# 1275468127/Medical-SAM2

Measured on AMD Instinct MI355X. Metric: slices/sec @1024^2 (Hiera-S), higher is better.
Workload: dtype bf16; 1 GPU; configs[1]: sam2_hiera_s 2D (train_2d SAM2 sub-sequence, forward), b=4 x 1024x1024 per GPU, 16-entry memory bank with 4 sampled memories per slice, one click per slice; forward_image -> memory_attention -> prompt encoder -> mask decoder -> memory encoder; hip_graph=True, weights=random name-keyed init

## Files before the change

include/msam2_hip.h:

```cpp
#ifndef MSAM2_HIP_H
#define MSAM2_HIP_H

#include <stddef.h>
#include <stdint.h>

#ifdef __cplusplus
extern "C" {
#endif

const char* msam2_last_error(void);

int msam2_version(void);

int msam2_operand_is_fp16(void);

int msam2_graph_begin(void* stream);

int msam2_graph_end(void* stream, void** graph_exec_out);

int msam2_graph_launch(void* graph_exec, void* stream);

int msam2_graph_destroy(void* graph_exec);

int msam2_event_create(void** ev);
// ... 71 lines not shown
int msam2_bilinear_upsample(const float* x, float* y, int64_t planes, int64_t h, int64_t w, int64_t H, int64_t W, void* stream);

int msam2_sine_pos_2d(float* out, int64_t h, int64_t w, int64_t C, float temperature, void* stream);

int msam2_fourier_pe_grid(float* out, const float* gauss, int64_t h, int64_t w, int64_t C, void* stream);

int msam2_hiera_pos_embed(float* out, const float* pos_embed, const float* pos_embed_window, int64_t C, int64_t bh, int64_t bw, int64_t h, int64_t w, int64_t window, void* stream);

int msam2_aa_downsample(const float* x, float* y, int64_t planes, int64_t H, int64_t W, int64_t factor, float in_scale, float in_bias, void* stream);

int msam2_gate_rows(float* x, const float* score, float value, int64_t B, int64_t row_len, void* stream);

int msam2_any_positive(const float* x, float* out, int64_t B, int64_t row_len, void* stream);

int msam2_image_prep(const uint8_t* img_hwc, float* out_chw, int64_t H, int64_t W, int64_t S, const float* mean3, const float* std3, void* stream);

int msam2_non_overlap(const float* masks, float* out, int64_t n_obj, int64_t pixels, void* stream);

int msam2_seg_counts(const float* pred, const float* gt, const float* thresholds, int64_t n_thresholds, int64_t planes, int64_t pixels, int* counts, void* stream);

int msam2_im2col_patch7x7s4(const float* img, void* out, int64_t B, int64_t S, void* stream);

int msam2_patch_embed7x7s4(const float* img, const void* w_perm, const float* bias, const float* pos, float* out, int64_t B, int64_t S, int64_t E, void* stream);

int msam2_im2col3x3s2(const void* x, void* out, int64_t B, int64_t H, int64_t W, int64_t C, int64_t ld, void* stream);

int msam2_conv3x3s2_ln_gelu(const void* x, int in_is_16bit, const float* weight, const float* bias, const float* ln_w, const float* ln_b, void* y, int64_t B, int64_t H, int64_t W, int64_t Cin, int64_t Cout, int mask_mode, float mask_scale, float mask_bias, void* stream);

int msam2_dwconv7x7_ln(const float* x, const float* weight_tap_major, const float* bias, const float* ln_w, const float* ln_b, void* y, int64_t B, int64_t H, int64_t W, int64_t C, void* stream);

int msam2_convt2x2_shuffle(const void* gemm_out, const float* bias, const void* skip, const float* ln_w, const float* ln_b, void* y, int64_t B, int64_t h, int64_t w, int64_t C, void* stream);

int msam2_convt2x2_shuffle_f32skip(const void* gemm_out, const float* bias, const float* skip, const float* ln_w, const float* ln_b, void* y, int64_t B, int64_t h, int64_t w, int64_t C, void* stream);

int msam2_convt2x2_shuffle_shared(const void* gemm_out, const float* bias, const void* skip, int skip_is_16bit, const float* ln_w, const float* ln_b, void* y, int64_t B, int64_t h, int64_t w, int64_t C, int64_t skip_batch_stride, void* stream);

int msam2_hyper_masks(const float* hyper, const void* upscaled, float* masks, int64_t n, int64_t K, int64_t P, int64_t C, void* stream);

int msam2_prompt_points(const float* xy, const int* labels, const float* gauss, const float* point_emb, const float* not_a_point, float* out, int64_t n_points, int64_t C, float image_size, void* stream);

int msam2_prompt_points_padded(const float* xy, const int* labels, const float* gauss, const float* point_emb, const float* not_a_point, float* out, int64_t n_sets, int64_t P, int64_t n_pad, int64_t C, float image_size, void* stream);

int msam2_select_mask(const float* masks, const float* ious, const float* obj_scores, float* low_res, int* sel, float* iou_sel, int64_t n, int64_t P, int multimask, int dynamic_stability, float delta, float thresh, void* stream);

int msam2_gather_rows(const float* x, const int* sel, float* y, int64_t n, int64_t T, int64_t C, int64_t offset, void* stream);

int msam2_obj_ptr_mix(float* ptr, const float* obj_scores, const float* no_obj_ptr, int64_t n, int64_t C, void* stream);

int msam2_space_to_depth(const void* x, int in_is_16bit, void* out, int64_t B, int64_t H, int64_t W, int64_t C, int64_t k, int64_t ld, void* stream);

int msam2_token_mlp3(const float* hs, int64_t hs_batch_stride, int64_t hs_token_stride, const int* token_index, const void* w1, const float* b1, const void* w2, const float* b2, const void* w3, const float* b3, const int* out_dim, const int* sigmoid_flag, float* out, int64_t G, int64_t B, int64_t C, void* stream);

int msam2_token_mlp3_packed(const float* hs, int64_t hs_batch_stride, int64_t hs_token_stride, const int* token_index, const void* w1, const float* b1, const void* w2, const float* b2, const void* w3, const float* b3, const int* out_dim, const int* sigmoid_flag, float* out, const int* out_offset, const int* out_stride, int64_t G, int64_t B, int64_t C, void* stream);

size_t msam2_cc_workspace_bytes(int64_t N, int64_t H, int64_t W);

int msam2_cc_label(const uint8_t* img, int32_t* labels, int32_t* counts, int64_t N, int64_t H, int64_t W, void* workspace, size_t workspace_bytes, void* stream);

size_t msam2_fill_holes_workspace_bytes(int64_t N, int64_t H, int64_t W);

int msam2_fill_components(float* mask, int64_t N, int64_t H, int64_t W, int max_area, float threshold, int above, float fill_value, void* workspace, size_t workspace_bytes, void* stream);

int msam2_fill_holes(float* mask, int64_t N, int64_t H, int64_t W, int max_area, void* workspace, size_t workspace_bytes, void* stream);

int msam2_transpose16(const void* in, int64_t ldi, void* out, int64_t ldo, int64_t rows, int64_t cols, void* stream);

int msam2_gemm_tt(const void* A, int64_t lda, const void* B, int64_t ldb, float* C, int64_t ldc, float* a_colsum, int64_t M, int64_t N, int64_t K, void* stream);

int msam2_gemm_tt_acc(const void* A, int64_t lda, const void* B, int64_t ldb, float* C, int64_t ldc, float* a_colsum, int64_t M, int64_t N, int64_t K, void* stream);

int msam2_colsum(const void* x, int x_is_16bit, int64_t ldx, float* out, int64_t rows, int64_t cols, void* stream);

int msam2_act_bwd(const void* pre, int pre_is_16bit, const void* dy, int dy_is_16bit, void* out, int64_t n, int act, void* stream);

int msam2_layernorm_bwd(const float* x, int64_t ldx, const void* dy, int dy_is_16bit, int64_t ldd, const float* gamma, float* dx, int64_t ldo, float* dgamma, float* dbeta, int64_t rows, int64_t C, float eps, const float* add, int64_t ld_add, void* stream);

int msam2_softmax_rows(const float* s, int64_t ld_s, void* p, int64_t ld_p, int64_t rows, int64_t cols, float scale, void* stream);

int msam2_softmax_bwd_rows(const void* p, int64_t ld_p, const float* dp, int64_t ld_dp, void* ds, int64_t ld_ds, int64_t rows, int64_t cols, float scale, void* stream);

int msam2_convt2x2_gather(const void* gemm_out, const float* bias, const void* skip, float* z, int64_t B, int64_t h, int64_t w, int64_t C, void* stream);

int msam2_convt2x2_scatter_grad(const void* dz, int dz_is_16bit, void* dg, int64_t B, int64_t h, int64_t w, int64_t C, void* stream);

int msam2_dwconv7x7(const float* x, const float* w_tap_major, const float* bias, float* y, int64_t B, int64_t H, int64_t W, int64_t C, int flip, void* stream);

int msam2_dwconv7x7_wgrad(const float* x, const float* dy, float* dw_tap_major, int64_t B, int64_t H, int64_t W, int64_t C, void* stream);

int msam2_col2im3x3s2(const float* dcols, int64_t ld, float* dx, int64_t B, int64_t H, int64_t W, int64_t C, void* stream);

int msam2_bilinear_upsample_bwd(const float* dy, float* dx, int64_t planes, int64_t h, int64_t w, int64_t H, int64_t W, void* stream);

int msam2_bce_logits(const float* logits, const float* target, float* dlogits, float* loss, int64_t n, float pos_weight, void* stream);

int msam2_adam_step(float* param, const float* grad, float* exp_avg, float* exp_avg_sq, int64_t n, float lr, float beta1, float beta2, float eps, int64_t step, void* stream);

int msam2_adam_step_multi(void* const* params, const void* const* grads, void* const* exp_avg, void* const* exp_avg_sq, const int64_t* numel, int64_t count, float lr, float beta1, float beta2, float eps, int64_t step, float grad_scale, float weight_decay, void* step_counter, void* skipped_counter, void* stream);

int msam2_attention_small_bwd(const void* q, int64_t q_bs, int64_t q_ts, const void* k, int64_t k_bs, int64_t k_ts, const void* v, int64_t v_bs, int64_t v_ts, const float* d_o, float* dq, float* dk, float* dv, int64_t B, int64_t H, int64_t Lq, int64_t Lk, int64_t D, float scale, void* stream);

int msam2_maxpool2x2_bwd(const void* x, int x_is_16bit, int64_t ldx, const float* dy, int64_t lddy, float* dx, int64_t lddx, int64_t B, int64_t H, int64_t W, int64_t C, void* stream);

int msam2_window_move(void* img, int64_t ld_img, void* win, const void* fill, int64_t B, int64_t H, int64_t W, int64_t heads, int64_t D, int64_t ws, int elem_bytes, int to_windows, void* stream);

int msam2_window_unpartition_cvt(void* img16, int64_t ld_img, const float* win, int64_t B, int64_t H, int64_t W, int64_t heads, int64_t D, int64_t ws, void* stream);

// ... 95 lines not shown
```

medical-sam2_amd/_lib.py:

```python
from __future__ import annotations

import ctypes
import os
import subprocess

_HERE = os.path.dirname(os.path.abspath(__file__))
LIB_PATH = os.environ.get("MSAM2_LIB_PATH") or os.path.join(_HERE, "libmsam2_hip.so")

c_p = ctypes.c_void_p
c_i = ctypes.c_int
c_l = ctypes.c_int64
c_f = ctypes.c_float
c_z = ctypes.c_size_t
c_d = ctypes.c_double

SIGNATURES = {
    "msam2_version": (c_i, []),
    "msam2_last_error": (ctypes.c_char_p, []),
    "msam2_operand_is_fp16": (c_i, []),
    "msam2_gemm": (c_i, [c_p, c_l, c_p, c_l, c_p, c_p, c_p, c_l, c_i, c_l, c_p, c_l, c_i, c_l, c_l, c_l, c_i, c_p]),
    "msam2_gemm_pool2x2": (c_i, [c_p, c_l, c_p, c_l, c_p, c_p, c_l, c_l, c_l, c_l, c_l, c_l, c_p]),
    "msam2_gemm_qkv_pool2x2": (c_i, [c_p, c_l, c_p, c_l, c_p, c_p, c_l, c_p, c_l, c_l, c_l, c_l, c_l, c_l, c_l, c_p]),
    "msam2_gemm_tokens": (c_i, [c_p, c_l, c_p, c_l, c_p, c_l, c_p, c_p, c_l, c_p, c_l, c_i, c_l, c_l, c_l, c_i, c_p]),
    "msam2_gemm_rope": (c_i, [c_p, c_l, c_p, c_l, c_p, c_p, c_l, c_l, c_l, c_l, c_p, c_p, c_l, c_l, c_l, c_l, c_l, c_p]),
    "msam2_gemm_residual_layernorm_supported": (c_i, [c_l, c_l]),
    "msam2_gemm_residual_layernorm": (c_i, [c_p, c_l, c_p, c_l, c_p, c_p, c_l, c_p, c_l, c_p, c_p, c_f, c_p, c_l, c_l, c_l, c_l, c_p]),
    "msam2_ln_mlp_residual_supported": (c_i, [c_l]),
    "msam2_mlp_fused_permute_w2": (c_i, [c_p, c_p, c_l, c_l, c_p]),
    "msam2_ln_mlp_residual_fwd": (c_i, [c_p, c_l, c_l, c_p, c_p, c_f, c_p, c_p, c_p, c_p, c_p, c_p]),
    "msam2_ln_mlp_residual_fwd_dual": (c_i, [c_p, c_l, c_l, c_p, c_p, c_f, c_p, c_p, c_p, c_p, c_p, c_p, c_p]),
    "msam2_proj_ln_mlp_residual_supported": (c_i, [c_l]),
    "msam2_mlp_fused_permute_w1": (c_i, [c_p, c_p, c_l, c_l, c_p]),
    "msam2_proj_ln_mlp_residual_fwd": (c_i, [c_p, c_p, c_p, c_p, c_l, c_l, c_p, c_p, c_f, c_p, c_p, c_p, c_p, c_p, c_p, c_p, c_p, c_f, c_p, c_p]),
    "msam2_layernorm": (c_i, [c_p, c_i, c_l, c_p, c_p, c_p, c_i, c_l, c_l, c_l, c_f, c_i, c_p]),
    "msam2_layernorm_dual": (c_i, [c_p, c_l, c_p, c_p, c_p, c_l, c_p, c_l, c_l, c_l, c_f, c_p]),
    "msam2_attention_workspace_bytes": (c_z, [c_l, c_l, c_l, c_l, c_i]),
    "msam2_attention_fwd": (c_i, [c_p, c_p, c_p, c_p, c_p, c_p, c_p, c_p, c_l, c_l, c_l, c_l, c_l, c_f, c_i, c_p, c_z, c_p]),
    "msam2_attention_fwd_lse": (c_i, [c_p, c_p, c_p, c_p, c_p, c_p, c_p, c_p, c_l, c_l, c_l, c_l, c_l, c_f, c_i, c_p, c_z, c_p, c_p]),
    "msam2_attention_fwd_lse_dropout": (c_i, [c_p, c_p, c_p, c_p, c_p, c_p, c_p, c_p, c_l, c_l, c_l, c_l, c_l, c_f, c_i, c_p, c_z, c_p, c_f,
                                              ctypes.c_uint64, ctypes.c_uint64, c_p, c_p]),
    "msam2_attention_kv64_fwd": (c_i, [c_p, c_p, c_p, c_p, c_p, c_p, c_p, c_p, c_l, c_l, c_l, c_l, c_f, c_i, c_p, c_z, c_p]),
    "msam2_attention_kv64_partial": (c_i, [c_p, c_p, c_p, c_p, c_p, c_p, c_l, c_l, c_l, c_l, c_f, c_i, c_i, c_i, c_p, c_z, c_p]),
    "msam2_attention_kv64_dyn_fwd": (c_i, [c_p, c_p, c_p, c_p, c_p, c_p, c_p, c_p, c_l, c_l, c_l, c_l, c_p, c_f, c_i, c_p, c_z, c_p]),
    "msam2_attention_kv64_dyn_partial": (c_i, [c_p, c_p, c_p, c_p, c_p, c_p, c_l, c_l, c_l, c_l, c_p, c_f, c_i, c_i, c_i, c_p, c_z, c_p]),
    "msam2_attention_effective_splits": (c_i, [c_l, c_i]),
    "msam2_attention_merge": (c_i, [c_p, c_p, c_l, c_l, c_l, c_l, c_l, c_i, c_p, c_z, c_p]),
    "msam2_window_attention_fwd": (c_i, [c_p, c_l, c_l, c_l, c_l, c_l, c_p, c_p, c_l, c_l, c_l, c_l, c_l, c_p, c_p, c_p, c_l, c_l,
                                         c_l, c_l, c_l, c_f, c_p]),
    "msam2_window_qkv_attention_supported": (c_i, [c_l, c_l, c_l, c_l, c_i, c_l, c_l]),
    "msam2_window_qkv_attention_fwd": (c_i, [c_p, c_p, c_p, c_p, c_l, c_l, c_l, c_l, c_l, c_l, c_i, c_f, c_p]),
    "msam2_attention_small_fwd": (c_i, [c_p, c_l, c_l, c_p, c_l, c_l, c_p, c_l, c_l, c_p, c_l, c_l, c_l, c_l, c_l, c_l, c_l, c_f,
                                        c_p]),
    "msam2_add_cast": (c_i, [c_p, c_i, c_l, c_l, c_p, c_i, c_l, c_l, c_f, c_p, c_i, c_l, c_l, c_l, c_p]),
    "msam2_maxpool2x2": (c_i, [c_p, c_i, c_l, c_p, c_i, c_l, c_l, c_l, c_l, c_l, c_p]),
    "msam2_upsample2x_add": (c_i, [c_p, c_p, c_l, c_l, c_l, c_l, c_p]),
    "msam2_rope_table": (c_i, [c_p, c_p, c_l, c_l, c_f, c_p]),
    "msam2_rope_inplace": (c_i, [c_p, c_l, c_l, c_l, c_l, c_l, c_l, c_l, c_p, c_p, c_p]),
    "msam2_bilinear_upsample": (c_i, [c_p, c_p, c_l, c_l, c_l, c_l, c_l, c_p]),
    "msam2_sine_pos_2d": (c_i, [c_p, c_l, c_l, c_l, c_f, c_p]),
    "msam2_fourier_pe_grid": (c_i, [c_p, c_p, c_l, c_l, c_l, c_p]),
    "msam2_hiera_pos_embed": (c_i, [c_p, c_p, c_p, c_l, c_l, c_l, c_l, c_l, c_l, c_p]),
    "msam2_im2col_patch7x7s4": (c_i, [c_p, c_p, c_l, c_l, c_p]),
    "msam2_patch_embed7x7s4": (c_i, [c_p, c_p, c_p, c_p, c_p, c_l, c_l, c_l, c_p]),
    "msam2_im2col3x3s2": (c_i, [c_p, c_p, c_l, c_l, c_l, c_l, c_l, c_p]),
    "msam2_conv3x3s2_ln_gelu": (c_i, [c_p, c_i, c_p, c_p, c_p, c_p, c_p, c_l, c_l, c_l, c_l, c_l, c_i, c_f, c_f, c_p]),
    "msam2_dwconv7x7_ln": (c_i, [c_p, c_p, c_p, c_p, c_p, c_p, c_l, c_l, c_l, c_l, c_p]),
    "msam2_convt2x2_shuffle": (c_i, [c_p, c_p, c_p, c_p, c_p, c_p, c_l, c_l, c_l, c_l, c_p]),
    "msam2_convt2x2_shuffle_f32skip": (c_i, [c_p, c_p, c_p, c_p, c_p, c_p, c_l, c_l, c_l, c_l, c_p]),
    "msam2_space_to_depth": (c_i, [c_p, c_i, c_p, c_l, c_l, c_l, c_l, c_l, c_l, c_p]),
    "msam2_aa_downsample": (c_i, [c_p, c_p, c_l, c_l, c_l, c_l, c_f, c_f, c_p]),
    "msam2_gate_rows": (c_i, [c_p, c_p, c_f, c_l, c_l, c_p]),
    "msam2_any_positive": (c_i, [c_p, c_p, c_l, c_l, c_p]),
    "msam2_transpose16": (c_i, [c_p, c_l, c_p, c_l, c_l, c_l, c_p]),
    "msam2_colsum": (c_i, [c_p, c_i, c_l, c_p, c_l, c_l, c_p]),
    "msam2_act_bwd": (c_i, [c_p, c_i, c_p, c_i, c_p, c_l, c_i, c_p]),
    "msam2_layernorm_bwd": (c_i, [c_p, c_l, c_p, c_i, c_l, c_p, c_p, c_l, c_p, c_p, c_l, c_l, c_f, c_p, c_l, c_p]),
    "msam2_softmax_rows": (c_i, [c_p, c_l, c_p, c_l, c_l, c_l, c_f, c_p]),
    "msam2_softmax_bwd_rows": (c_i, [c_p, c_l, c_p, c_l, c_p, c_l, c_l, c_l, c_f, c_p]),
    "msam2_convt2x2_gather": (c_i, [c_p, c_p, c_p, c_p, c_l, c_l, c_l, c_l, c_p]),
    "msam2_convt2x2_scatter_grad": (c_i, [c_p, c_i, c_p, c_l, c_l, c_l, c_l, c_p]),
    "msam2_bce_logits": (c_i, [c_p, c_p, c_p, c_p, c_l, c_f, c_p]),
    "msam2_attention_bwd_workspace_bytes": (c_z, [c_l, c_l, c_l, c_l]),
    "msam2_attention_bwd": (c_i, [c_p, c_p, c_p, c_p, c_p, c_p, c_p, c_p, c_p, c_p, c_p, c_p, c_p, c_p, c_p, c_p, c_p, c_p, c_z,
                                  c_l, c_l, c_l, c_l, c_l, c_f, c_p]),
    "msam2_attention_bwd_dropout": (c_i, [c_p, c_p, c_p, c_p, c_p, c_p, c_p, c_p, c_p, c_p, c_p, c_p, c_p, c_p, c_p, c_p, c_p, c_p, c_z,
                                          c_l, c_l, c_l, c_l, c_l, c_f, c_f, ctypes.c_uint64, ctypes.c_uint64, c_p, c_p]),
    "msam2_dwconv7x7": (c_i, [c_p, c_p, c_p, c_p, c_l, c_l, c_l, c_l, c_i, c_p]),
    "msam2_dwconv7x7_wgrad": (c_i, [c_p, c_p, c_p, c_l, c_l, c_l, c_l, c_p]),
    "msam2_col2im3x3s2": (c_i, [c_p, c_l, c_p, c_l, c_l, c_l, c_l, c_p]),
    "msam2_gemm_nt": (c_i, [c_p, c_l, c_p, c_l, c_p, c_p, c_l, c_p, c_l, c_i, c_l, c_l, c_l, c_p]),
    "msam2_gemm_tt": (c_i, [c_p, c_l, c_p, c_l, c_p, c_l, c_p, c_l, c_l, c_l, c_p]),
    "msam2_window_unpartition_cvt": (c_i, [c_p, c_l, c_p, c_l, c_l, c_l, c_l, c_l, c_l, c_p]),
    "msam2_window_pad_colsum": (c_i, [c_p, c_p, c_l, c_l, c_l, c_l, c_l, c_l, c_p]),
    "msam2_gemm_tt_acc": (c_i, [c_p, c_l, c_p, c_l, c_p, c_l, c_p, c_l, c_l, c_l, c_p]),
    "msam2_bilinear_upsample_bwd": (c_i, [c_p, c_p, c_l, c_l, c_l, c_l, c_l, c_p]),
    "msam2_maxpool2x2_bwd": (c_i, [c_p, c_i, c_l, c_p, c_l, c_p, c_l, c_l, c_l, c_l, c_l, c_p]),
    "msam2_window_move": (c_i, [c_p, c_l, c_p, c_p, c_l, c_l, c_l, c_l, c_l, c_l, c_i, c_i, c_p]),
    "msam2_sumpool2x2": (c_i, [c_p, c_p, c_l, c_l, c_l, c_l, c_p]),
    "msam2_hiera_pos_embed_bwd": (c_i, [c_p, c_p, c_p, c_l, c_l, c_l, c_l, c_l, c_l, c_p, c_z, c_p]),
    "msam2_hiera_pos_embed_bwd_workspace_bytes": (c_z, [c_l, c_l, c_l, c_l]),
    "msam2_dropout": (c_i, [c_p, c_i, c_l, c_p, c_l, c_p, c_i, c_l, c_l, c_l, c_f, ctypes.c_uint64, ctypes.c_uint64, c_p, c_p]),
    "msam2_counter_bump": (c_i, [c_p, c_p, c_p]),
    "msam2_adam_step": (c_i, [c_p, c_p, c_p, c_p, c_l, c_f, c_f, c_f, c_f, c_l, c_p]),
    "msam2_adam_step_multi": (c_i, [c_p, c_p, c_p, c_p, c_p, c_l, c_f, c_f, c_f, c_f, c_l, c_f, c_f, c_p, c_p, c_p]),
    "msam2_attention_small_bwd": (c_i, [c_p, c_l, c_l, c_p, c_l, c_l, c_p, c_l, c_l, c_p, c_p, c_p, c_p, c_l, c_l, c_l, c_l, c_l, c_f, c_p]),
    "msam2_seg_counts": (c_i, [c_p, c_p, c_p, c_l, c_l, c_l, c_p, c_p]),
    "msam2_non_overlap": (c_i, [c_p, c_p, c_l, c_l, c_p]),
    "msam2_token_mlp3": (c_i, [c_p, c_l, c_l, c_p, c_p, c_p, c_p, c_p, c_p, c_p, c_p, c_p, c_p, c_l, c_l, c_l, c_p]),
    "msam2_hyper_masks": (c_i, [c_p, c_p, c_p, c_l, c_l, c_l, c_l, c_p]),
    "msam2_prompt_points": (c_i, [c_p, c_p, c_p, c_p, c_p, c_p, c_l, c_l, c_f, c_p]),
    "msam2_prompt_points_padded": (c_i, [c_p, c_p, c_p, c_p, c_p, c_p, c_l, c_l, c_l, c_l, c_f, c_p]),
    "msam2_token_mlp3_packed": (c_i, [c_p, c_l, c_l, c_p, c_p, c_p, c_p, c_p, c_p, c_p, c_p, c_p, c_p, c_p, c_p, c_l, c_l, c_l, c_p]),
    "msam2_select_mask": (c_i, [c_p, c_p, c_p, c_p, c_p, c_p, c_l, c_l, c_i, c_i, c_f, c_f, c_p]),
    "msam2_gather_rows": (c_i, [c_p, c_p, c_p, c_l, c_l, c_l, c_l, c_p]),
    "msam2_obj_ptr_mix": (c_i, [c_p, c_p, c_p, c_l, c_l, c_p]),
    "msam2_convt2x2_shuffle_shared": (c_i, [c_p, c_p, c_p, c_i, c_p, c_p, c_p, c_l, c_l, c_l, c_l, c_l, c_p]),
    "msam2_mask_stats_workspace_bytes": (c_z, [c_l]),
    "msam2_mask_stats": (c_i, [c_p, c_l, c_l, c_l, c_l, c_l, c_f, c_f, c_f, c_p, c_p, c_p, c_z, c_p]),
# ... 82 lines not shown
```

medical-sam2_amd/modeling/memory.py:

```python
from __future__ import annotations

import copy
import math
from typing import Optional, Tuple

import torch
import torch.nn as nn

from .. import ops
from .common import OP16, F32, WeightCache, attn_splits, nchw_view, to_bf16, tokens_of, v_f32, w_bf16
from .encoder import MLP


import os as _os
_FUSED_ROPE = _os.environ.get("MSAM2_NO_FUSED_ROPE") is None
_FOLD_V = _os.environ.get("MSAM2_NO_VALUE_FOLD") is None
_BATCH_K_PROJ = _os.environ.get("MSAM2_BATCHED_KPROJ") is not None


class LayerNorm2d(nn.Module):

    def __init__(self, num_channels: int, eps: float = 1e-6) -> None:
        super().__init__()
        self.weight = nn.Parameter(torch.ones(num_channels))
        self.bias = nn.Parameter(torch.zeros(num_channels))
        self.eps = eps

    def forward(self, x: torch.Tensor) -> torch.Tensor:
        B, C, H, W = x.shape
        y = ops.layernorm(tokens_of(x), self.weight.detach().float(), self.bias.detach().float(), self.eps, out_dtype=F32)
        return nchw_view(y, B, H, W)


class Attention(nn.Module):

    def __init__(self, embedding_dim: int, num_heads: int, downsample_rate: int = 1, dropout: float = 0.0, kv_in_dim: int = None):
        super().__init__()
        self.embedding_dim = embedding_dim
        self.kv_in_dim = kv_in_dim if kv_in_dim is not None else embedding_dim
        self.internal_dim = embedding_dim // downsample_rate
        self.num_heads = num_heads
        assert self.internal_dim % num_heads == 0, "num_heads must divide embedding_dim."
        self.q_proj = nn.Linear(embedding_dim, self.internal_dim)
        self.k_proj = nn.Linear(self.kv_in_dim, self.internal_dim)
        self.v_proj = nn.Linear(self.kv_in_dim, self.internal_dim)
        self.out_proj = nn.Linear(self.internal_dim, embedding_dim)
        self.dropout_p = dropout
        self._wc = WeightCache()

    def proj(self, which: str, x_bf16: torch.Tensor) -> torch.Tensor:
        lin = getattr(self, which + "_proj")
        return ops.gemm(x_bf16, w_bf16(self._wc, which + "w", lin.weight), v_f32(self._wc, which + "b", lin.bias))

    def out(self, o_bf16: torch.Tensor, residual: Optional[torch.Tensor], out_dtype=F32) -> torch.Tensor:
        return ops.gemm(o_bf16, w_bf16(self._wc, "ow", self.out_proj.weight), v_f32(self._wc, "ob", self.out_proj.bias),
                        residual=residual, out_dtype=out_dtype)

    def core(self, q: torch.Tensor, k: torch.Tensor, v: torch.Tensor) -> torch.Tensor:
        B, Lq, C = q.shape
        D = C // self.num_heads
        if D in (16, 32):
            return ops.attention_small(q, k, v, self.num_heads).reshape(B * Lq, C)
        H = self.num_heads
        sp = lambda t: t.view(B, t.shape[1], H, D).permute(0, 2, 1, 3)
        o = ops.attention(sp(q), sp(k), sp(v), splits=attn_splits(B, H, Lq, k.shape[1]))
        return o.permute(0, 2, 1, 3).reshape(B * Lq, C)

    def forward(self, q: torch.Tensor, k: torch.Tensor, v: torch.Tensor) -> torch.Tensor:
        assert not (self.training and self.dropout_p > 0.0), "attention dropout (train mode) is outside the forward hot path"
        B, Lq, _ = q.shape
# ... 228 lines not shown
        L, B, C = curr.shape
        from .. import autograd as ag
        if ag.active(self) and key_count is None:
            pos = curr_pos if (curr_pos is not None and self.pos_enc_at_input) else torch.zeros_like(curr)
            return ag.memory_attention(self, curr, pos, memory, memory_pos, num_obj_ptr_tokens)
        drop = self.next_dropout()
        if drop is not None:
            from .. import backward as bwd
            assert key_count is None, "padded memory banks are an inference-path feature"
            zero = torch.zeros_like(curr) if curr_pos is None or not self.pos_enc_at_input else curr_pos
            return bwd.memory_attention_forward_saved(self, curr, zero, memory, memory_pos, num_obj_ptr_tokens, dropout=drop)[0]
        use_pos = self.pos_enc_at_input and curr_pos is not None
        x = ops.add_cast(curr.transpose(0, 1), curr_pos.transpose(0, 1) if use_pos else None, 0.1, F32).reshape(B * L, C)
        mem_bf = memory.transpose(0, 1)
        mem_k = ops.add_cast(mem_bf, memory_pos.transpose(0, 1), 1.0, OP16)
        mem_v = ops.add_cast(mem_bf, None, 1.0, OP16)
        kk_all = self._project_all_keys(mem_k, B, L, num_obj_ptr_tokens)
        for i, layer in enumerate(self.layers):
            x = layer.run(x, mem_k, mem_v, B, L, num_obj_ptr_tokens, key_count, None if kk_all is None else kk_all[:, :, i])
        y = ops.layernorm(x, v_f32(self._wc, "nw", self.norm.weight), v_f32(self._wc, "nb", self.norm.bias), self.norm.eps,
                          out_dtype=F32)
        return y.view(B, L, C).transpose(0, 1)


class MaskDownSampler(nn.Module):

    def __init__(self, embed_dim=256, kernel_size=4, stride=4, padding=0, total_stride=16, activation=nn.GELU):
        super().__init__()
        assert (kernel_size, stride, padding, total_stride) == (3, 2, 1, 16) and activation is nn.GELU, \
            "HIP path implements the YAML's k3/s2/p1 mask down-sampler"
        num_layers = int(math.log2(total_stride) // math.log2(stride))
        self.encoder = nn.Sequential()
        cin = 1
        for _ in range(num_layers):
            cout = cin * (stride ** 2)
            self.encoder.append(nn.Conv2d(cin, cout, kernel_size=kernel_size, stride=stride, padding=padding))
            self.encoder.append(LayerNorm2d(cout))
            self.encoder.append(activation())
            cin = cout
        self.encoder.append(nn.Conv2d(cin, embed_dim, kernel_size=1))
        self._wc = WeightCache()

    def run(self, mask: torch.Tensor, mode: int, scale: float, bias: float) -> torch.Tensor:
        n, _, S, _ = mask.shape
        wc, enc = self._wc, self.encoder
        f = lambda key, p: v_f32(wc, key, p)
        h = mask.to(F32).contiguous().reshape(n * S * S, 1)
        conv, ln = enc[0], enc[1]
        h = ops.conv3x3s2_ln_gelu(h, n, S, S, wc.get("cw0", [conv.weight], lambda: conv.weight.detach().float().contiguous()),
                                  f("cb0", conv.bias), f("lw0", ln.weight), f("lb0", ln.bias), mode, scale, bias)
        side = S // 2
        for j in range(1, 4):
            conv, ln = enc[3 * j], enc[3 * j + 1]
            cols = ops.im2col3x3s2(h, n, side, side)

            def pack(c=conv, ld=cols.shape[1]):
                w = c.weight.detach().permute(0, 2, 3, 1).reshape(c.weight.shape[0], -1)
                out = torch.zeros(w.shape[0], ld, dtype=OP16, device=w.device)
                out[:, : w.shape[1]] = w.to(OP16)
                return out
            g = ops.gemm(cols, wc.get(f"cw{j}", [conv.weight], pack), f(f"cb{j}", conv.bias), out_dtype=F32)
            h = ops.layernorm(g, f(f"lw{j}", ln.weight), f(f"lb{j}", ln.bias), ln.eps, act=ops.ACT_GELU)
            side //= 2
        return ops.gemm(h, w_bf16(wc, "pw", enc[12].weight), f("pb", enc[12].bias), out_dtype=F32)

    def forward(self, x: torch.Tensor) -> torch.Tensor:
        n, _, S, _ = x.shape
        return nchw_view(self.run(x, 0, 0.0, 0.0), n, S // 16, S // 16)


class CXBlock(nn.Module):

    def __init__(self, dim, kernel_size=7, padding=3, drop_path=0.0, layer_scale_init_value=1e-6, use_dwconv=True):
        super().__init__()
        assert kernel_size == 7 and padding == 3 and use_dwconv and drop_path == 0.0 and layer_scale_init_value > 0
        self.dwconv = nn.Conv2d(dim, dim, kernel_size=7, padding=3, groups=dim)
        self.norm = LayerNorm2d(dim, eps=1e-6)
        self.pwconv1 = nn.Linear(dim, 4 * dim)
        self.act = nn.GELU()
        self.pwconv2 = nn.Linear(4 * dim, dim)
        self.gamma = nn.Parameter(layer_scale_init_value * torch.ones(dim), requires_grad=True)
        self._wc = WeightCache()

    def run(self, x: torch.Tensor, n: int, H: int, W: int) -> torch.Tensor:
        wc = self._wc
        C = x.shape[1]
        wt = wc.get("dw", [self.dwconv.weight], lambda: self.dwconv.weight.detach().reshape(C, 49).t().float().contiguous())
        h = ops.dwconv7x7_ln(x, n, H, W, wt, v_f32(wc, "dwb", self.dwconv.bias), v_f32(wc, "lw", self.norm.weight),
                             v_f32(wc, "lb", self.norm.bias))
        h = ops.gemm(h, w_bf16(wc, "w1", self.pwconv1.weight), v_f32(wc, "b1", self.pwconv1.bias), act=ops.ACT_GELU)
        return ops.gemm(h, w_bf16(wc, "w2", self.pwconv2.weight), v_f32(wc, "b2", self.pwconv2.bias),
                        colscale=v_f32(wc, "g", self.gamma), residual=x, out_dtype=F32)

    def forward(self, x: torch.Tensor) -> torch.Tensor:
        n, C, H, W = x.shape
        return nchw_view(self.run(tokens_of(x.to(F32)), n, H, W), n, H, W)


class Fuser(nn.Module):

    def __init__(self, layer, num_layers, dim=None, input_projection=False):
        super().__init__()
        assert not input_projection, "SAM2 configs use no input projection in the fuser"
        self.proj = nn.Identity()
        self.layers = nn.ModuleList([copy.deepcopy(layer) for _ in range(num_layers)])

    def run(self, x, n, H, W):
        for layer in self.layers:
            x = layer.run(x, n, H, W)
        return x

    def forward(self, x: torch.Tensor) -> torch.Tensor:
        n, C, H, W = x.shape
        return nchw_view(self.run(tokens_of(x.to(F32)), n, H, W), n, H, W)

# ... 31 lines not shown
```

medical-sam2_amd/ops.py:

```python
from __future__ import annotations

import ctypes
import math
from typing import Optional, Tuple

import torch

from ._lib import check, lib

OP16 = torch.float16 if lib().msam2_operand_is_fp16() else torch.bfloat16

F32 = torch.float32
ACT_NONE, ACT_GELU, ACT_RELU, ACT_SIGMOID = 0, 1, 2, 3


def _stream() -> int:
    return torch.cuda.current_stream().cuda_stream


def _p(t: Optional[torch.Tensor]):
    return None if t is None else t.data_ptr()


def _is_bf16(t: torch.Tensor) -> int:
# ... 466 lines not shown
    out = torch.empty(h * w, C, dtype=F32, device=pos_embed.device)
    check(lib().msam2_hiera_pos_embed(_p(out), _p(pos_embed.contiguous()), _p(pos_embed_window.contiguous()), C, bh, bw, h, w,
                                      pos_embed_window.shape[-1], _stream()))
    return out


def im2col_patch(img: torch.Tensor) -> torch.Tensor:
    _req(img.dtype == F32 and img.is_contiguous() and img.shape[1] == 3 and img.shape[2] == img.shape[3], "im2col_patch: [B,3,S,S] fp32")
    B, _, S, _ = img.shape
    out = torch.empty(B * (S // 4) ** 2, 160, dtype=OP16, device=img.device)
    check(lib().msam2_im2col_patch7x7s4(_p(img), _p(out), B, S, _stream()))
    return out


def patch_embed_supported(S: int, E: int) -> bool:
    So = S // 4
    return S % 4 == 0 and So % 32 == 0 and E <= 128


def patch_embed(img: torch.Tensor, w_perm: torch.Tensor, bias: torch.Tensor, pos: Optional[torch.Tensor] = None) -> torch.Tensor:
    _req(img.dtype == F32 and img.is_contiguous() and img.shape[1] == 3 and img.shape[2] == img.shape[3], "patch_embed: [B,3,S,S] fp32")
    B, _, S, _ = img.shape
    E = bias.shape[0]
    _req(patch_embed_supported(S, E), "patch_embed: unsupported size (use im2col_patch + gemm)")
    _req(w_perm.dtype == OP16 and w_perm.is_contiguous() and tuple(w_perm.shape) == ((E + 31) // 32 * 32, 176), "patch_embed: w_perm [ceil32(E), 176] 16-bit")
    _req(bias.dtype == F32 and bias.is_contiguous(), "patch_embed: fp32 bias")
    if pos is not None:
        _req(pos.dtype == F32 and pos.is_contiguous() and tuple(pos.shape) == ((S // 4) ** 2, E), "patch_embed: pos fp32 [(S/4)^2, E]")
    out = torch.empty(B * (S // 4) ** 2, E, dtype=F32, device=img.device)
    check(lib().msam2_patch_embed7x7s4(_p(img), _p(w_perm), _p(bias), _p(pos), _p(out), B, S, E, _stream()))
    return out


def im2col3x3s2(x: torch.Tensor, B: int, H: int, W: int) -> torch.Tensor:
    C = x.shape[-1]
    _req(x.dtype == OP16 and x.is_contiguous(), "im2col3x3s2: 16-bit contiguous NHWC")
    ld = (9 * C + 7) // 8 * 8
    out = torch.empty(B * (H // 2) * (W // 2), ld, dtype=OP16, device=x.device)
    check(lib().msam2_im2col3x3s2(_p(x), _p(out), B, H, W, C, ld, _stream()))
    return out


def conv3x3s2_ln_gelu(x: torch.Tensor, B: int, H: int, W: int, weight, bias, ln_w, ln_b, mask_mode: int = 0,
                      mask_scale: float = 0.0, mask_bias: float = 0.0) -> torch.Tensor:
    cout, cin = weight.shape[0], weight.shape[1]
    _req(x.dtype == (F32 if cin == 1 else OP16) and x.is_contiguous() and x.numel() == B * H * W * cin,
         "conv3x3s2_ln_gelu: contiguous NHWC [B*H*W, cin], fp32 for cin = 1, 16-bit otherwise")
    _req(all(t.dtype == F32 and t.is_contiguous() for t in (weight, bias, ln_w, ln_b)) and tuple(weight.shape[2:]) == (3, 3)
         and bias.numel() == cout and ln_w.numel() == cout and ln_b.numel() == cout, "conv3x3s2_ln_gelu: fp32 contiguous [cout, cin, 3, 3] weight, [cout] vectors")
    y = torch.empty(B * (H // 2) * (W // 2), cout, dtype=OP16, device=x.device)
    check(lib().msam2_conv3x3s2_ln_gelu(_p(x), _is_bf16(x), _p(weight), _p(bias), _p(ln_w), _p(ln_b), _p(y), B, H, W, cin, cout,
                                        mask_mode, mask_scale, mask_bias, _stream()))
    return y


def dwconv7x7_ln(x: torch.Tensor, B: int, H: int, W: int, w_tap_major, bias, ln_w, ln_b) -> torch.Tensor:
    _req(x.dtype == F32 and x.is_contiguous(), "dwconv7x7_ln: fp32 contiguous NHWC")
    C = x.shape[-1]
    y = torch.empty(B * H * W, C, dtype=OP16, device=x.device)
    check(lib().msam2_dwconv7x7_ln(_p(x), _p(w_tap_major), _p(bias), _p(ln_w), _p(ln_b), _p(y), B, H, W, C, _stream()))
    return y


def convt2x2_shuffle(g: torch.Tensor, bias, skip: torch.Tensor, ln_w, ln_b, B: int, h: int, w: int) -> torch.Tensor:
    C = g.shape[1] // 4
    _req(g.dtype == OP16 and skip.dtype in (OP16, F32) and g.is_contiguous() and skip.is_contiguous(), "convt2x2_shuffle: contiguous 16-bit g, 16-bit / fp32 skip")
    y = torch.empty(B * 4 * h * w, C, dtype=OP16, device=g.device)
    if skip.dtype == F32:
        _req(C in (32, 64), "convt2x2_shuffle: fp32 skip features need C = 32 / 64")
        check(lib().msam2_convt2x2_shuffle_f32skip(_p(g), _p(bias), _p(skip), _p(ln_w), _p(ln_b), _p(y), B, h, w, C, _stream()))
    else:
        check(lib().msam2_convt2x2_shuffle(_p(g), _p(bias), _p(skip), _p(ln_w), _p(ln_b), _p(y), B, h, w, C, _stream()))
    return y


def convt2x2_shuffle_shared(g: torch.Tensor, bias, skip: torch.Tensor, ln_w, ln_b, B: int, h: int, w: int) -> torch.Tensor:
    C = g.shape[1] // 4
    _req(g.dtype == OP16 and skip.dtype in (OP16, F32) and g.is_contiguous() and skip.is_contiguous(), "convt2x2_shuffle_shared: contiguous 16-bit g, 16-bit / fp32 skip")
    _req(skip.numel() == 4 * h * w * C, "convt2x2_shuffle_shared: skip must be one [4hw, C] map")
    y = torch.empty(B * 4 * h * w, C, dtype=OP16, device=g.device)
    check(lib().msam2_convt2x2_shuffle_shared(_p(g), _p(bias), _p(skip), _is_bf16(skip), _p(ln_w), _p(ln_b), _p(y), B, h, w, C, 0, _stream()))
    return y


def hyper_masks(hyper: torch.Tensor, up: torch.Tensor, n: int, P: int) -> torch.Tensor:
    K, C = hyper.shape[1], hyper.shape[2]
    _req(hyper.dtype == F32 and hyper.shape[0] == n, "hyper_masks: hyper must be fp32 [n, K, C]")
    _req(up.dtype == OP16 and up.is_contiguous() and up.numel() == n * P * C, "hyper_masks: up must be 16-bit contiguous [n*P, C]")
    masks = torch.empty(n, K, P, dtype=F32, device=up.device)
    check(lib().msam2_hyper_masks(_p(hyper.contiguous()), _p(up), _p(masks), n, K, P, C, _stream()))
    return masks


def prompt_points(xy: torch.Tensor, labels: torch.Tensor, gauss, point_emb, not_a_point, image_size: float, n_pad: int = 0) -> torch.Tensor:
    n, P = labels.shape
    C = point_emb.shape[1]
    out = torch.empty(n, P + n_pad, C, dtype=F32, device=xy.device)
    check(lib().msam2_prompt_points_padded(_p(xy.contiguous()), _p(labels.contiguous()), _p(gauss), _p(point_emb), _p(not_a_point), _p(out),
                                           n, P, n_pad, C, float(image_size), _stream()))
    return out


def select_mask(masks: torch.Tensor, ious: torch.Tensor, obj: torch.Tensor, multimask: bool, dynamic: bool, delta: float,
                thresh: float):
    n, K, h, w = masks.shape
    low = torch.empty(n, 1, h, w, dtype=F32, device=masks.device)
# ... 721 lines not shown
```

Baseline: 763.5 slices/s.

## Fuse mask-downsampler conv3x3s2 im2col, MFMA GEMM, LayerNorm and GELU into one kernel

Adds an MFMA kernel for the memory encoder's mask downsampler. It gathers 3x3 stride-2 patches straight from NHWC input, accumulates in registers with double-buffered fragment loads, then applies bias, LayerNorm and GELU from an LDS tile before writing 16-bit output. Stages 2-4 (4->16, 16->64, 64->256 channels) use it by default instead of im2col + GEMM + LayerNorm, which removes the im2col buffer and the fp32 GEMM output round trip. The cost is a more complex kernel whose GELU uses a polynomial erf approximation, so rounding may differ slightly from the old path.

```diff
diff --git a/include/msam2_hip.h b/include/msam2_hip.h
--- a/include/msam2_hip.h
+++ b/include/msam2_hip.h
@@ -147,6 +147,10 @@
 int msam2_token_mlp3(const float* hs, int64_t hs_batch_stride, int64_t hs_token_stride, const int* token_index, const void* w1, const float* b1, const void* w2, const float* b2, const void* w3, const float* b3, const int* out_dim, const int* sigmoid_flag, float* out, int64_t G, int64_t B, int64_t C, void* stream);
 
 int msam2_token_mlp3_packed(const float* hs, int64_t hs_batch_stride, int64_t hs_token_stride, const int* token_index, const void* w1, const float* b1, const void* w2, const float* b2, const void* w3, const float* b3, const int* out_dim, const int* sigmoid_flag, float* out, const int* out_offset, const int* out_stride, int64_t G, int64_t B, int64_t C, void* stream);
+
+int msam2_conv3x3s2_mfma_ln_gelu_supported(int64_t cin, int64_t cout);
+
+int msam2_conv3x3s2_mfma_ln_gelu(const void* x, const void* w_packed, int64_t ldw, const float* bias, const float* ln_w, const float* ln_b, float eps, void* y, int64_t ldy, int64_t B, int64_t H, int64_t W, int64_t cin, int64_t cout, void* stream);
 
 size_t msam2_cc_workspace_bytes(int64_t N, int64_t H, int64_t W);
 
diff --git a/medical-sam2_amd/_lib.py b/medical-sam2_amd/_lib.py
--- a/medical-sam2_amd/_lib.py
+++ b/medical-sam2_amd/_lib.py
@@ -64,6 +64,8 @@
     "msam2_patch_embed7x7s4": (c_i, [c_p, c_p, c_p, c_p, c_p, c_l, c_l, c_l, c_p]),
     "msam2_im2col3x3s2": (c_i, [c_p, c_p, c_l, c_l, c_l, c_l, c_l, c_p]),
     "msam2_conv3x3s2_ln_gelu": (c_i, [c_p, c_i, c_p, c_p, c_p, c_p, c_p, c_l, c_l, c_l, c_l, c_l, c_i, c_f, c_f, c_p]),
+    "msam2_conv3x3s2_mfma_ln_gelu_supported": (c_i, [c_l, c_l]),
+    "msam2_conv3x3s2_mfma_ln_gelu": (c_i, [c_p, c_p, c_l, c_p, c_p, c_p, c_f, c_p, c_l, c_l, c_l, c_l, c_l, c_l, c_p]),
     "msam2_dwconv7x7_ln": (c_i, [c_p, c_p, c_p, c_p, c_p, c_p, c_l, c_l, c_l, c_l, c_p]),
     "msam2_convt2x2_shuffle": (c_i, [c_p, c_p, c_p, c_p, c_p, c_p, c_l, c_l, c_l, c_l, c_p]),
     "msam2_convt2x2_shuffle_f32skip": (c_i, [c_p, c_p, c_p, c_p, c_p, c_p, c_l, c_l, c_l, c_l, c_p]),
diff --git a/medical-sam2_amd/csrc/conv_mfma.hip b/medical-sam2_amd/csrc/conv_mfma.hip
--- /dev/null
+++ b/medical-sam2_amd/csrc/conv_mfma.hip
@@ -0,0 +1,265 @@
+#include "common.h"
+
+struct ConvLnParams {
+  const op16* X;
+  const op16* W;
+  const float* bias;
+  const float* ln_w;
+  const float* ln_b;
+  op16* Y;
+  int64_t ldw, ldy;
+  int B, H, Wd, M;
+  float eps;
+};
+
+template <int CPL, int LPR, int C>
+__device__ __forceinline__ void ln_row_stats(const float (&v)[CPL][4], float eps, float& mean, float& rstd) {
+#pragma clang fp contract(off)
+  float s = 0.f;
+#pragma unroll
+  for (int j = 0; j < CPL; ++j)
+#pragma unroll
+    for (int e = 0; e < 4; ++e) s += v[j][e];
+#pragma unroll
+  for (int o = LPR / 2; o > 0; o >>= 1) s += __shfl_xor(s, o, 64);
+  mean = s / C;
+  const float d0 = v[0][0] - mean, d1 = v[0][1] - mean;
+  float q = d1 * d1;
+  q = __builtin_fmaf(d0, d0, q);
+#pragma unroll
+  for (int i = 2; i < CPL * 4; ++i) {
+    const float d = v[i >> 2][i & 3] - mean;
+    q = __builtin_fmaf(d, d, q);
+  }
+#pragma unroll
+  for (int o = LPR / 2; o > 0; o >>= 1) q += __shfl_xor(q, o, 64);
+  rstd = 1.0f / sqrtf(q / C + eps);
+}
+
+__device__ __forceinline__ float ln_gelu_value(float x, float mean, float rstd, float w, float b) {
+#pragma clang fp contract(off)
+  const float u = __builtin_fmaf(w, rstd * (x - mean), b);
+  const float ab = fabsf(u);
+  const float ax = ab * 0.70710678118654752440f;
+  const float t = __builtin_amdgcn_rcpf(__builtin_fmaf(ax, 0.3275911f, 1.0f));
+  float poly = __builtin_fmaf(t, 1.061405429f, -1.453152027f);
+  poly = __builtin_fmaf(t, poly, 1.421413741f);
+  poly = __builtin_fmaf(t, poly, -0.284496736f);
+  poly = __builtin_fmaf(t, poly, 0.254829592f);
+  poly = t * poly;
+  const float ex = __builtin_amdgcn_exp2f((ax * ax) * (-1.44269504088896340736f));
+  return __builtin_fmaf(-(ab * 0.5f), poly * ex, fmaxf(u, 0.f));
+}
+
+template <int CIN, int COUT, int WR, int WC, bool SKINNY>
+__global__ __launch_bounds__(WR* WC * 64) void conv3x3s2_mfma_kernel(ConvLnParams p) {
+#if defined(__HIP_DEVICE_COMPILE__)
+  constexpr int NW = WR * WC, BM = WR * 32;
+  constexpr int TNW = COUT / WC;
+  constexpr int FN = TNW >= 32 ? TNW / 32 : 1;
+  constexpr int KR = 9 * CIN, KP = (KR + 7) / 8 * 8;
+  constexpr int KSTEPS = SKINNY ? KP / 16 : (KP + 31) / 32 * 2;
+  constexpr int PER = (KSTEPS + 3) / 4;
+  constexpr int G = CIN == 16 ? 5 : 4;
+  constexpr int NG = (KSTEPS + G - 1) / G;
+  constexpr int TLD = COUT + 4;
+  constexpr int NCH = COUT / 4;
+  constexpr int LPR = NCH < 16 ? NCH : 16;
+  constexpr int CPL = NCH / LPR;
+  constexpr int RPW = 64 / LPR;
+  constexpr int PASSES = BM / (NW * RPW);
+  static_assert(CIN == 4 || CIN % 16 == 0, "eight consecutive k: 8 channels of one tap, or two taps x 4 channels");
+  static_assert(COUT % WC == 0 && (TNW % 32 == 0 || (WC == 1 && COUT == 16)) && BM % (NW * RPW) == 0 && NCH % LPR == 0 && (LPR & (LPR - 1)) == 0,
+                "wave tiling");
+  static_assert(!SKINNY || KP % 16 == 0, "gemm_skinny_kernel serves K % 16 == 0 only");
+  extern __shared__ __attribute__((aligned(16))) unsigned char lds[];
+  float* tile = reinterpret_cast<float*>(lds);
+  const int tid = threadIdx.x;
+  const int wave = __builtin_amdgcn_readfirstlane(tid >> 6), lane = tid & 63;
+  const int wr = wave / WC, wc = wave % WC;
+  const int r = lane & 31, h = lane >> 5;
+  const int64_t m0 = (int64_t)xcd_tile_order(blockIdx.x, gridDim.x) * BM;
+  if (m0 >= p.M) return;
+
+  const unsigned Ho = (unsigned)p.H >> 1, Wo = (unsigned)p.Wd >> 1;
+  const unsigned m = (unsigned)min(m0 + wr * 32 + r, (int64_t)p.M - 1);
+  const unsigned t1 = m / Wo, ox = m - t1 * Wo;
+  const unsigned b = t1 / Ho, oy = t1 - b * Ho;
+  const int y0 = 2 * (int)oy - 1, x0 = 2 * (int)ox - 1;
+  const op16* xb = p.X + (int64_t)b * p.H * p.Wd * CIN;
+
+  auto load_a = [&](int ks) -> op16x8 {
+    op16x8 o;
+    if constexpr (CIN >= 16) {
+      const int tap = (16 * ks) / CIN, c = (16 * ks) % CIN + 8 * h;
+      const int ty = tap < 9 ? tap / 3 : 0, tx = tap < 9 ? tap % 3 : 0;
+      const int y = y0 + ty, x = x0 + tx;
+      const bool in = tap < 9 && y >= 0 && y < p.H && x >= 0 && x < p.Wd;
+      const op16x8 v = *reinterpret_cast<const op16x8*>(xb + ((int64_t)min(max(y, 0), p.H - 1) * p.Wd + min(max(x, 0), p.Wd - 1)) * CIN + c);
+#pragma unroll
+      for (int e = 0; e < 8; ++e) o[e] = in ? v[e] : (op16)0.f;
+    } else {
+#pragma unroll
+      for (int q = 0; q < 2; ++q) {
+        const int tap = 4 * ks + 2 * h + q;
+        const int tc = min(tap, 8), ty = tc / 3, tx = tc - 3 * ty;
+        const int y = y0 + ty, x = x0 + tx;
+        const bool in = tap < 9 && y >= 0 && y < p.H && x >= 0 && x < p.Wd;
+        const op16x4 v = *reinterpret_cast<const op16x4*>(xb + ((int64_t)min(max(y, 0), p.H - 1) * p.Wd + min(max(x, 0), p.Wd - 1)) * CIN);
+#pragma unroll
+        for (int e = 0; e < 4; ++e) o[4 * q + e] = in ? v[e] : (op16)0.f;
+      }
+    }
+    return o;
+  };
+  const op16* wrow[FN];
+  bool w_in[FN];
+#pragma unroll
+  for (int j = 0; j < FN; ++j) {
+    const int n = wc * TNW + j * 32 + r;
+    w_in[j] = n < COUT;
+    wrow[j] = p.W + (int64_t)min(n, COUT - 1) * p.ldw;
+  }
+  auto load_w = [&](int ks, int j) -> op16x8 {
+    const int k0 = 16 * ks + 8 * h;
+    const op16x8 v = *reinterpret_cast<const op16x8*>(wrow[j] + min(k0, KP - 8));
+    const bool in = w_in[j] && k0 < KP;
+    op16x8 o;
+#pragma unroll
+    for (int e = 0; e < 8; ++e) o[e] = in ? v[e] : (op16)0.f;
+    return o;
+  };
+
+  float bias_j[FN];
+#pragma unroll
+  for (int j = 0; j < FN; ++j) bias_j[j] = p.bias[min(wc * TNW + j * 32 + r, COUT - 1)];
+
+  f32x16 acc[FN], tot[FN];
+  zero_acc(acc);
+  zero_acc(tot);
+  op16x8 af[2][G], wf[2][G][FN];
+  auto load_group = [&](int g, int buf) {
+#pragma unroll
+    for (int s = 0; s < G; ++s) {
+      const int ks = min(g * G + s, KSTEPS - 1);
+      af[buf][s] = load_a(ks);
+#pragma unroll
+      for (int j = 0; j < FN; ++j) wf[buf][s][j] = load_w(ks, j);
+    }
+  };
+  load_group(0, 0);
+#pragma unroll
+  for (int g = 0; g < NG; ++g) {
+    if (g + 1 < NG) load_group(g + 1, (g + 1) & 1);
+#pragma unroll
+    for (int s = 0; s < G; ++s) {
+      const int ks = g * G + s;
+      if (ks < KSTEPS) {
+#pragma unroll
+        for (int j = 0; j < FN; ++j) acc[j] = MSAM2_MFMA_32x32x16(af[g & 1][s], wf[g & 1][s][j], acc[j], 0, 0, 0);
+        if constexpr (SKINNY) {
+          if ((ks + 1) % PER == 0 || ks == KSTEPS - 1) {
+#pragma unroll
+            for (int j = 0; j < FN; ++j)
+#pragma unroll
+              for (int e = 0; e < 16; ++e) {
+                tot[j][e] = ks < PER ? acc[j][e] : tot[j][e] + acc[j][e];
+                acc[j][e] = 0.f;
+              }
+          }
+        }
+      }
+    }
+  }
+  if constexpr (SKINNY) {
+#pragma unroll
+    for (int q = (KSTEPS + PER - 1) / PER; q < 4; ++q)
+#pragma unroll
+      for (int j = 0; j < FN; ++j)
+#pragma unroll
+        for (int e = 0; e < 16; ++e) tot[j][e] = tot[j][e] + acc[j][e];
+  }
+
+  const int ll = lane % LPR;
+  f32x4 ww[CPL], bb[CPL];
+#pragma unroll
+  for (int j = 0; j < CPL; ++j) {
+    ww[j] = *reinterpret_cast<const f32x4*>(p.ln_w + (ll + LPR * j) * 4);
+    bb[j] = *reinterpret_cast<const f32x4*>(p.ln_b + (ll + LPR * j) * 4);
+  }
+#pragma unroll
+  for (int j = 0; j < FN; ++j) {
+    const int n = wc * TNW + j * 32 + r;
+    if (n < COUT) {
+#pragma unroll
+      for (int e = 0; e < 16; ++e) tile[(wr * 32 + s_frag_key(e, h)) * TLD + n] = (SKINNY ? tot[j][e] : acc[j][e]) + bias_j[j];
+    }
+  }
+  __syncthreads();
+#pragma unroll
+  for (int ps = 0; ps < PASSES; ++ps) {
+    const int trow = (ps * NW + wave) * RPW + lane / LPR;
+    const int64_t grow = m0 + trow;
+    float v[CPL][4];
+#pragma unroll
+    for (int j = 0; j < CPL; ++j) {
+      const f32x4 t = *reinterpret_cast<const f32x4*>(tile + trow * TLD + (ll + LPR * j) * 4);
+#pragma unroll
+      for (int e = 0; e < 4; ++e) v[j][e] = t[e];
+    }
+    float mean, rstd;
+    ln_row_stats<CPL, LPR, COUT>(v, p.eps, mean, rstd);
+    if (grow < p.M) {
+      op16* yr = p.Y + grow * p.ldy;
+#pragma unroll
+      for (int j = 0; j < CPL; ++j) {
+        op16x4 o;
+#pragma unroll
+        for (int e = 0; e < 4; ++e) o[e] = f2out<op16>(ln_gelu_value(v[j][e], mean, rstd, ww[j][e], bb[j][e]));
+        *reinterpret_cast<op16x4*>(yr + (ll + LPR * j) * 4) = o;
+      }
+    }
+  }
+#endif
+}
+
+template <int CIN, int COUT, int WR, int WC>
+static void conv3x3s2_mfma_launch(const ConvLnParams& p, hipStream_t s) {
+  constexpr int LDS = WR * 32 * (COUT + 4) * 4;
+  const dim3 grid(cdiv(p.M, WR * 32)), block(WR * WC * 64);
+  if constexpr (((9 * CIN + 7) / 8 * 8) % 16 == 0) {
+    if (p.M <= 32) {
+      ensure_dyn_lds<conv3x3s2_mfma_kernel<CIN, COUT, WR, WC, true>>(LDS);
+      hipLaunchKernelGGL((conv3x3s2_mfma_kernel<CIN, COUT, WR, WC, true>), grid, block, LDS, s, p);
+      return;
+    }
+  }
+  ensure_dyn_lds<conv3x3s2_mfma_kernel<CIN, COUT, WR, WC, false>>(LDS);
+  hipLaunchKernelGGL((conv3x3s2_mfma_kernel<CIN, COUT, WR, WC, false>), grid, block, LDS, s, p);
+}
+
+extern "C" int msam2_conv3x3s2_mfma_ln_gelu_supported(int64_t cin, int64_t cout) {
+  return ((cin == 4 && cout == 16) || (cin == 16 && cout == 64) || (cin == 64 && cout == 256)) ? 1 : 0;
+}
+
+extern "C" int msam2_conv3x3s2_mfma_ln_gelu(const void* x, const void* w_packed, int64_t ldw, const float* bias, const float* ln_w, const float* ln_b,
+                                            float eps, void* y, int64_t ldy, int64_t B, int64_t H, int64_t W, int64_t cin, int64_t cout, void* stream) {
+  MSAM2_REQUIRE(x && w_packed && bias && ln_w && ln_b && y, "conv3x3s2_mfma_ln_gelu: null operand");
+  MSAM2_REQUIRE(msam2_conv3x3s2_mfma_ln_gelu_supported(cin, cout), "conv3x3s2_mfma_ln_gelu: cin=%lld cout=%lld is not built (4->16, 16->64, 64->256)",
+                (long long)cin, (long long)cout);
+  MSAM2_REQUIRE(B > 0 && H > 0 && W > 0 && H % 2 == 0 && W % 2 == 0, "conv3x3s2_mfma_ln_gelu: B=%lld H=%lld W=%lld (even H, W)", (long long)B,
+                (long long)H, (long long)W);
+  MSAM2_REQUIRE(B * H * W * cin < (1ll << 31), "conv3x3s2_mfma_ln_gelu: more than 2^31 input elements");
+  MSAM2_REQUIRE(ldw % 8 == 0 && ldw >= (9 * cin + 7) / 8 * 8 && ldy % 4 == 0 && ldy >= cout,
+                "conv3x3s2_mfma_ln_gelu: ldw must be a multiple of 8, >= ceil8(9 cin); ldy a multiple of 4, >= cout");
+  MSAM2_REQUIRE(vec_ok(8, 2, x, w_packed) && vec_ok(4, 4, (const void*)bias, (const void*)ln_w, (const void*)ln_b) && vec_ok(4, 2, y),
+                "conv3x3s2_mfma_ln_gelu: x, w_packed, bias, ln_w, ln_b must be 16-byte aligned, y 8-byte");
+  ConvLnParams p;
+  p.X = (const op16*)x; p.W = (const op16*)w_packed; p.bias = bias; p.ln_w = ln_w; p.ln_b = ln_b; p.Y = (op16*)y;
+  p.ldw = ldw; p.ldy = ldy; p.B = (int)B; p.H = (int)H; p.Wd = (int)W; p.M = (int)(B * (H / 2) * (W / 2)); p.eps = eps;
+  hipStream_t s = (hipStream_t)stream;
+  if (cin == 4) conv3x3s2_mfma_launch<4, 16, 4, 1>(p, s);
+  else if (cin == 16) conv3x3s2_mfma_launch<16, 64, 4, 1>(p, s);
+  else conv3x3s2_mfma_launch<64, 256, 2, 4>(p, s);
+  return msam2_check_launch("conv3x3s2_mfma_ln_gelu");
+}
diff --git a/medical-sam2_amd/modeling/memory.py b/medical-sam2_amd/modeling/memory.py
--- a/medical-sam2_amd/modeling/memory.py
+++ b/medical-sam2_amd/modeling/memory.py
@@ -16,6 +16,18 @@
 _FUSED_ROPE = _os.environ.get("MSAM2_NO_FUSED_ROPE") is None
 _FOLD_V = _os.environ.get("MSAM2_NO_VALUE_FOLD") is None
 _BATCH_K_PROJ = _os.environ.get("MSAM2_BATCHED_KPROJ") is not None
+_FUSED_MASK_DS = _os.environ.get("MSAM2_NO_FUSED_MASK_DS") is None
+
+
+def _stage_list(text: str) -> frozenset:
+    return frozenset(int(k) for k in text.split(",") if k.strip())
+
+
+_FUSED_MASK_DS_STAGES = _stage_list(_os.environ.get("MSAM2_FUSED_MASK_DS_STAGES", "2,3,4"))
+
+
+def _mask_ds_dispatched(stage: int, cin: int, cout: int) -> bool:
+    return _FUSED_MASK_DS and stage in _FUSED_MASK_DS_STAGES and ops.conv3x3s2_mfma_ln_gelu_supported(cin, cout)
 
 
 class LayerNorm2d(nn.Module):
@@ -350,15 +362,19 @@
         side = S // 2
         for j in range(1, 4):
             conv, ln = enc[3 * j], enc[3 * j + 1]
-            cols = ops.im2col3x3s2(h, n, side, side)
-
-            def pack(c=conv, ld=cols.shape[1]):
+            cout, cin = conv.weight.shape[0], conv.weight.shape[1]
+
+            def pack(c=conv, ld=(9 * cin + 7) // 8 * 8):
                 w = c.weight.detach().permute(0, 2, 3, 1).reshape(c.weight.shape[0], -1)
                 out = torch.zeros(w.shape[0], ld, dtype=OP16, device=w.device)
                 out[:, : w.shape[1]] = w.to(OP16)
                 return out
-            g = ops.gemm(cols, wc.get(f"cw{j}", [conv.weight], pack), f(f"cb{j}", conv.bias), out_dtype=F32)
-            h = ops.layernorm(g, f(f"lw{j}", ln.weight), f(f"lb{j}", ln.bias), ln.eps, act=ops.ACT_GELU)
+            w = wc.get(f"cw{j}", [conv.weight], pack)
+            if _mask_ds_dispatched(j + 1, cin, cout):
+                h = ops.conv3x3s2_mfma_ln_gelu(h, n, side, side, w, f(f"cb{j}", conv.bias), f(f"lw{j}", ln.weight), f(f"lb{j}", ln.bias), ln.eps)
+            else:
+                g = ops.gemm(ops.im2col3x3s2(h, n, side, side), w, f(f"cb{j}", conv.bias), out_dtype=F32)
+                h = ops.layernorm(g, f(f"lw{j}", ln.weight), f(f"lb{j}", ln.bias), ln.eps, act=ops.ACT_GELU)
             side //= 2
         return ops.gemm(h, w_bf16(wc, "pw", enc[12].weight), f("pb", enc[12].bias), out_dtype=F32)
 
diff --git a/medical-sam2_amd/ops.py b/medical-sam2_amd/ops.py
--- a/medical-sam2_amd/ops.py
+++ b/medical-sam2_amd/ops.py
@@ -542,6 +542,28 @@
     check(lib().msam2_conv3x3s2_ln_gelu(_p(x), _is_bf16(x), _p(weight), _p(bias), _p(ln_w), _p(ln_b), _p(y), B, H, W, cin, cout,
                                         mask_mode, mask_scale, mask_bias, _stream()))
     return y
+
+
+def conv3x3s2_mfma_ln_gelu_supported(cin: int, cout: int) -> bool:
+    return bool(lib().msam2_conv3x3s2_mfma_ln_gelu_supported(cin, cout))
+
+
+def conv3x3s2_mfma_ln_gelu(x: torch.Tensor, B: int, H: int, W: int, w_packed: torch.Tensor, bias: torch.Tensor, ln_w: torch.Tensor,
+                           ln_b: torch.Tensor, eps: float, *, out: Optional[torch.Tensor] = None) -> torch.Tensor:
+    _req(x.dtype == OP16 and x.is_contiguous() and x.numel() % (B * H * W) == 0, "conv3x3s2_mfma_ln_gelu: 16-bit contiguous NHWC")
+    cin = x.numel() // (B * H * W)
+    _req(w_packed.dim() == 2 and w_packed.dtype == OP16 and w_packed.stride(1) == 1, "conv3x3s2_mfma_ln_gelu: w_packed must be 16-bit [cout, ld]")
+    cout = w_packed.shape[0]
+    _req(conv3x3s2_mfma_ln_gelu_supported(cin, cout), f"conv3x3s2_mfma_ln_gelu: {cin} -> {cout} channels is not built (4 -> 16, 16 -> 64, 64 -> 256)")
+    _req(w_packed.shape[1] >= (9 * cin + 7) // 8 * 8, "conv3x3s2_mfma_ln_gelu: w_packed rows hold ceil8(9 cin) columns")
+    _req(all(t.dtype == F32 and t.is_contiguous() and t.numel() == cout for t in (bias, ln_w, ln_b)), "conv3x3s2_mfma_ln_gelu: bias, ln_w, ln_b are fp32 [cout]")
+    M = B * (H // 2) * (W // 2)
+    if out is None:
+        out = torch.empty(M, cout, dtype=OP16, device=x.device)
+    _req(out.dtype == OP16 and out.shape == (M, cout) and out.stride(1) == 1, "conv3x3s2_mfma_ln_gelu: out must be 16-bit [M, cout], rows contiguous")
+    check(lib().msam2_conv3x3s2_mfma_ln_gelu(_p(x), _p(w_packed), w_packed.stride(0), _p(bias), _p(ln_w), _p(ln_b), float(eps), _p(out),
+                                             out.stride(0), B, H, W, cin, cout, _stream()))
+    return out
 
 
 def dwconv7x7_ln(x: torch.Tensor, B: int, H: int, W: int, w_tap_major, bias, ln_w, ln_b) -> torch.Tensor:
```

Measured after the change: 773.7 slices/s (median of 6 runs). +1.3%, better.
